# robotics-upo/social_force_window_planner

Measured on AMD Instinct MI355X. Metric: scored trajectories/sec (v x w samples x steps) @ N pedestrians; cmd_vel match, higher is better.
Workload: dtype f64

## Files before the change

include/sfw_hip.h:

```cpp
#ifndef SFW_HIP_H_
#define SFW_HIP_H_

#include <stdint.h>

#ifdef __cplusplus
extern "C" {
#endif

#define SFW_ABI_VERSION 2

typedef enum sfw_status {
  SFW_OK = 0,
  SFW_ERR_INVALID_ARG = -1,
  SFW_ERR_NO_DEVICE = -2,
  SFW_ERR_HIP = -3,
  SFW_ERR_STATE = -4,
  SFW_ERR_UNSUPPORTED = -5
} sfw_status;

#define SFW_COST_INVALID (-1.0)
#define SFW_COST_SKIPPED (-2.0)

#define SFW_ROBOT_ID_NONE INT32_MIN

// ... 128 lines not shown
int sfw_sequences_perturb_stage(sfw_handle h, const sfw_robot_state *rs, const sfw_perturb *p, int32_t n, int32_t K,
                                const int32_t *knot_step, const sfw_goal_args *args, int64_t index_base);
int sfw_score_perturbed(sfw_handle h, const sfw_robot_state *rs, const sfw_perturb *p, int32_t n, int32_t K,
                        const int32_t *knot_step, const sfw_goal_args *args, double *costs_out, sfw_best *best_out);
int sfw_sequences_knots(sfw_handle h, int64_t first, int64_t count, double *vx_out, double *vy_out, double *vtheta_out);
int sfw_sequences_normals(sfw_handle h, int64_t first, int64_t count, double *z_out);

#define SFW_ORG_NONE 0
#define SFW_ORG_REGISTER_1 1
#define SFW_ORG_REGISTER_2 2
#define SFW_ORG_FLAT 3
typedef struct sfw_plan_info {
  int32_t split_step;
  int32_t levels;
  int32_t chunks;
  int32_t organisation;
  int64_t classes;
  int64_t class_steps;
  int64_t samples;
  int64_t flat_samples;
  int64_t one_launch;
  int64_t rest_noise_unreproduced;
} sfw_plan_info;
int sfw_grid_plan_info(sfw_handle h, sfw_plan_info *out);
int sfw_plan_shared_prefix(const double *linvels, int32_t nv,
                           const double *angvels, int32_t nw, double vx0,
                           double vtheta0, double acc_x, double acc_theta,
                           double sim_time, int32_t num_steps,
                           int32_t n_agents, int32_t *level_ends,
                           int64_t *level_classes, int32_t cap,
                           int32_t *n_levels);
int sfw_plan_axis_classes(const double *targets, int32_t n, double v0, double a_max, double dt, int32_t max_p,
                          int32_t form, int32_t *counts, int32_t *classes, int32_t *n_levels, int32_t *closed_form);
int sfw_plan_row_blocks(const double *linvels, int32_t nv, const double *angvels, int32_t nw, double vx0,
                        double vtheta0, double acc_x, double acc_theta, double sim_time, int32_t num_steps,
                        int32_t n_agents, int32_t R, int32_t *row0);
#define SFW_K2_AUTO (-1)
#define SFW_K2_REGISTER 0
#define SFW_K2_FLAT 1
int sfw_set_k2_form(sfw_handle h, int32_t form);
int sfw_set_timing(sfw_handle h, int32_t enabled);
int sfw_last_launch_ms(sfw_handle h, int32_t which, float *ms_out);
int sfw_last_clock_ghz(sfw_handle h, double *ghz_out);
int sfw_grid_points(sfw_handle h, int64_t index, double *points_xyth,
                    int32_t points_cap, int32_t *n_points);
int sfw_grid_points_batch(sfw_handle h, int64_t first, int64_t count, double *points_xyth, int32_t *n_points);
int sfw_set_points_capture(sfw_handle h, int32_t enabled);
void *sfw_stream(sfw_handle h);

#define SFW_TERM_VEL 0
#define SFW_TERM_DISTANCE 1
#define SFW_TERM_ANGLE 2
#define SFW_TERM_COSTMAP 3
#define SFW_TERM_SOCIAL 4
#define SFW_N_TERMS 5
#define SFW_RESCORE_MAX_K 1024
typedef struct sfw_weights {
  double vel, distance, angle, costmap, social;
} sfw_weights;
int sfw_set_terms_capture(sfw_handle h, int32_t enabled);
int sfw_grid_rescore(sfw_handle h, const sfw_weights *w, int32_t K, sfw_best *best_out, double *costs_out);
int sfw_grid_terms(sfw_handle h, int64_t first, int64_t count, double *terms_out);

#define SFW_BLEND_MAX_L 16
typedef struct sfw_blend_stat {
  double lambda;
// ... 120 lines not shown
```

social_force_window_planner_amd/_abi.py:

```python
import ctypes as C

SFW_OK = 0
SFW_ERR_INVALID_ARG = -1
SFW_ERR_NO_DEVICE = -2
SFW_ERR_HIP = -3
SFW_ERR_STATE = -4
SFW_ERR_UNSUPPORTED = -5

SFW_COST_INVALID = -1.0
SFW_COST_SKIPPED = -2.0

SFW_PRECISION_F64 = 0
SFW_PRECISION_F32 = 1
SFW_PRECISION_F64_STRICT = 2

SFW_K2_AUTO, SFW_K2_REGISTER, SFW_K2_FLAT = -1, 0, 1
SFW_ORG_NONE, SFW_ORG_REGISTER_1, SFW_ORG_REGISTER_2, SFW_ORG_FLAT = 0, 1, 2, 3


class SfwParams(C.Structure):
    _fields_ = [
        ("max_vel_x", C.c_double),
        ("sim_time", C.c_double),
        ("sim_granularity", C.c_double),
# ... 104 lines not shown
class SfwPlanInfo(C.Structure):
    _fields_ = [("split_step", C.c_int32), ("levels", C.c_int32), ("chunks", C.c_int32), ("organisation", C.c_int32),
                ("classes", C.c_int64), ("class_steps", C.c_int64), ("samples", C.c_int64), ("flat_samples", C.c_int64),
                ("one_launch", C.c_int64), ("rest_noise_unreproduced", C.c_int64)]

    def as_dict(self):
        return {"split_step": self.split_step, "levels": self.levels, "chunks": self.chunks, "classes": self.classes,
                "class_steps": self.class_steps, "samples": self.samples, "organisation": self.organisation,
                "flat_samples": self.flat_samples, "one_launch": self.one_launch,
                "rest_noise_unreproduced": self.rest_noise_unreproduced}


EXPORTED_SYMBOLS = (
    "sfw_params_default",
    "sfw_abi_version",
    "sfw_create",
    "sfw_destroy",
    "sfw_set_params",
    "sfw_last_error",
    "sfw_set_costmap",
    "sfw_set_footprint",
    "sfw_set_agents",
    "sfw_score_grid",
    "sfw_score_one",
    "sfw_grid_stage",
    "sfw_grid_launch",
    "sfw_grid_sync",
    "sfw_grid_fetch",
    "sfw_grid_costs_view",
    "sfw_grid_plan_info",
    "sfw_plan_shared_prefix",
    "sfw_plan_row_blocks",
    "sfw_plan_axis_classes",
    "sfw_set_k2_form",
    "sfw_set_timing",
    "sfw_last_launch_ms",
    "sfw_last_clock_ghz",
    "sfw_grid_points",
    "sfw_grid_points_batch",
    "sfw_set_points_capture",
    "sfw_stream",
    "sfw_multi_create",
    "sfw_multi_destroy",
    "sfw_multi_last_error",
    "sfw_multi_describe",
    "sfw_multi_ranks",
    "sfw_multi_rank_handle",
    "sfw_multi_set_params",
    "sfw_multi_set_costmap",
    "sfw_multi_set_footprint",
    "sfw_multi_set_agents",
    "sfw_multi_score_grid",
    "sfw_multi_rank_rows",
    "sfw_multi_last_us",
    "sfw_multi_grid_points",
    "sfw_batch_create",
    "sfw_batch_destroy",
    "sfw_batch_last_error",
    "sfw_batch_size",
    "sfw_batch_member",
    "sfw_batch_launch",
    "sfw_batch_fetch",
    "sfw_batch_score_grid",
    "sfw_batch_describe",
    "sfw_batch_last_us",
    "sfw_set_terms_capture",
# ... 121 lines not shown
```

social_force_window_planner_amd/csrc/sfw_capi.hip:

```cpp

#include "sfw_device.h"

#include <dlfcn.h>
#include <link.h>

#include <algorithm>
#include <chrono>
#include <cmath>
#include <condition_variable>
#include <functional>
#include <mutex>
#include <thread>
#include <cstdio>
#include <cstdlib>
#include <cstring>
#include <limits>
#include <new>
#include <string>
#include <vector>

namespace {

template <typename T> struct dev_buf {
  T *p = nullptr;
// ... 32 lines not shown
    return hipEventSynchronize(done);
  }
  hipError_t reserve(size_t bytes) {
    hipError_t e = wait();
    if (e != hipSuccess) return e;
    if (!done && (e = hipEventCreateWithFlags(&done, hipEventDisableTiming)) != hipSuccess) return e;
    if (bytes <= cap) return hipSuccess;
    if (p) (void)hipHostFree(p);
    p = nullptr;
    cap = 0;
    const size_t want = bytes + bytes / 4 + 256;
    e = hipHostMalloc(reinterpret_cast<void **>(&p), want, hipHostMallocDefault);
    if (e == hipSuccess) cap = want;
    return e;
  }
  hipError_t mark(hipStream_t s) {
    pending = true;
    return hipEventRecord(done, s);
  }
  void release() {
    (void)wait();
    if (p) (void)hipHostFree(p);
    if (done) (void)hipEventDestroy(done);
    p = nullptr;
    cap = 0;
    done = nullptr;
  }
};

struct level_tables {
  int32_t n_row = 0, n_col = 0;
  size_t o_row_rep = 0, o_col_rep = 0;
  size_t o_row_src = 0, o_col_src = 0;
};
struct chunk_plan {
  std::vector<level_tables> lv;
  size_t o_row_cls = 0;
};

struct map_geometry {
  uint32_t size_x, size_y;
  double origin_x, origin_y, resolution;
};

struct agent_set {
  std::vector<char> blob;
  size_t ao_vel = 0, ao_cst = 0, ao_obs = 0, ao_grp = 0, ao_off = 0, ao_mem = 0;
  int A = 0, O = 0, NG = 0, n_grp_mem = 0;
  bool person_pinned = false;
  std::vector<std::pair<int32_t, int32_t>> rest_pairs;
};

}

struct sfw_planner_s {
  struct config {
    int n_cu = SFW_DEFAULT_CUS, n_xcd = SFW_DEFAULT_CUS / SFW_CUS_PER_XCD;
    std::vector<int> prefix_env;
    bool pin_rest_on = true;
    long spin_us = 20000;
    bool arena_direct_on = true;
    size_t mirror_max_bytes = size_t(64) << 20;
    int obs_tasks_force = -1;
    size_t table_budget_bytes = size_t(8) << 30;
    bool owns_streams = true;
    bool batch_member = false;
  } cfg;

  struct switches {
    sfw_params params;
// ... 506 lines not shown
  return steps;
}

void plan_row_blocks(const std::vector<double> &lin, const std::vector<double> &ang, double vx0, double vth0, double acc_x,
                     double acc_theta, double dt, int S, int A, int R, int form, int cus, std::vector<int32_t> &row0) {
  const int64_t nv = static_cast<int64_t>(lin.size()), nw = static_cast<int64_t>(ang.size());
  row0.assign(static_cast<size_t>(R) + 1, 0);
  for (int r = 0; r <= R; ++r) row0[static_cast<size_t>(r)] = static_cast<int32_t>((static_cast<int64_t>(r) * nv) / R);
  if (R <= 1 || A < 2 || S < 2 || (nv / R) * nw < 4096) return;
  prefix_classes pc;
  classes_of_grid(pc, lin, ang, vx0, vth0, acc_x, acc_theta, dt, S);
  const std::vector<int> steps = choose_levels(pc, nv * nw, S, static_cast<double>(sfw_samples_per_wave(A, (nv / R) * nw, form, cus)), cus);
  if (steps.empty()) return;
  std::vector<double> w(static_cast<size_t>(nv), static_cast<double>(nw) * (S - steps.back()));
  int prev = 0;
  for (int p : steps) {
    const std::vector<int32_t> &rc = pc.rows.level(p);
    const double per_class = static_cast<double>(pc.n_cols_at(p)) * (p - prev);
    for (int64_t i = 0; i < nv; ++i)
      if (i == 0 || rc[static_cast<size_t>(i)] != rc[static_cast<size_t>(i - 1)]) w[static_cast<size_t>(i)] += per_class;
    prev = p;
  }
  double total = 0.0;
  for (double v : w) total += v;
  double run = 0.0;
  int r = 1;
  for (int64_t i = 0; i < nv && r < R; ++i) {
    run += w[static_cast<size_t>(i)];
    while (r < R && run >= total * r / R) row0[static_cast<size_t>(r++)] = static_cast<int32_t>(i + 1);
  }
  for (; r < R; ++r) row0[static_cast<size_t>(r)] = static_cast<int32_t>(nv);
}

int plan_prefix(sfw_handle h, int64_t chunk, int S) {
  h->st.prefix_steps.clear();
  h->st.prefix_chunks.clear();
  h->st.cls_ints.clear();
  h->st.cls_max = 0;
  h->st.prefix_class_steps = h->st.prefix_last_classes = 0;
  const int64_t T = static_cast<int64_t>(h->st.nv) * h->st.nw;
  const bool forced = !h->cfg.prefix_env.empty();
  if (h->st.list) return SFW_OK;
  if ((forced && h->cfg.prefix_env[0] == 0) || h->st.A < 2 || S < 2 || h->st.vy_samp != 0.0) return SFW_OK;
  if (!forced && T < 4096) return SFW_OK;
  const int64_t rows_per_chunk = chunk / h->st.nw;
  if (rows_per_chunk < 1) return SFW_OK;
  prefix_classes pc;
  classes_of_grid(pc, h->st.lin, h->st.ang, h->st.rs.vx, h->st.rs.vtheta, h->st.ga.acc_x, h->st.ga.acc_theta, h->live.params.sim_time / S, S,
                  static_cast<const axis_classes *>(h->shared_cols));
  const axis_classes &rc = pc.rows, &cc = *pc.cols;
  const std::vector<int32_t> &nr = pc.rows.n, &nc = pc.cols->n;
  auto level = [](const axis_classes &c, int p) -> const std::vector<int32_t> & { return c.level(p); };
  auto count_at = [](const std::vector<int32_t> &n, int p) { return n[std::min<size_t>(static_cast<size_t>(p), n.size()) - 1]; };
  std::vector<int> steps;
  if (forced) {
    for (int p : h->cfg.prefix_env)
      if (p >= 1 && p <= pc.max_p) steps.push_back(p);
  } else {
    steps = choose_levels(pc, T, S, static_cast<double>(sfw_samples_per_wave(h->st.A, std::min<int64_t>(T, rows_per_chunk * h->st.nw), h->live.k2_form, h->cfg.n_cu)), h->cfg.n_cu);
  }
  if (steps.empty()) return SFW_OK;
  const size_t n_lv = steps.size();

  std::vector<int32_t> ints;
  ints.swap(h->st.cls_ints);
  ints.clear();
  ints.reserve(static_cast<size_t>(2 * n_lv + 2) * static_cast<size_t>(h->st.nv + h->st.nw));
  auto append = [&](const std::vector<int32_t> &v) {
    const size_t o = ints.size();
    ints.insert(ints.end(), v.begin(), v.end());
    return o;
  };
  std::vector<int32_t> ids;
  auto relabel = [&ids](const std::vector<int32_t> &cls, int64_t i0, int64_t i1, std::vector<int32_t> &local,
                        std::vector<int32_t> &rep) {
    ids.assign(cls.size(), -1);
    local.clear();
    rep.clear();
    local.reserve(static_cast<size_t>(i1 - i0));
    rep.reserve(static_cast<size_t>(i1 - i0));
    for (int64_t i = i0; i < i1; ++i) {
      int32_t &id = ids[static_cast<size_t>(cls[static_cast<size_t>(i)])];
      if (id < 0) {
        id = static_cast<int32_t>(rep.size());
        rep.push_back(static_cast<int32_t>(i - i0));
      }
      local.push_back(id);
    }
  };
  struct axis_level { std::vector<int32_t> local, rep, src; };
  auto axis_levels = [&](const axis_classes &cls, int64_t i0, int64_t i1) {
    std::vector<axis_level> out(n_lv);
    for (size_t l = 0; l < n_lv; ++l) {
      relabel(level(cls, steps[l]), i0, i1, out[l].local, out[l].rep);
      if (l > 0) {
        out[l].src.reserve(out[l].rep.size());
        for (int32_t r : out[l].rep) out[l].src.push_back(out[l - 1].local[static_cast<size_t>(r)]);
      }
    }
    return out;
  };
  const std::vector<axis_level> cols = axis_levels(cc, 0, h->st.nw);
  std::vector<size_t> o_col_rep(n_lv), o_col_src(n_lv);
  for (size_t l = 0; l < n_lv; ++l) {
    o_col_rep[l] = append(cols[l].rep);
    o_col_src[l] = append(cols[l].src);
  }
  h->st.prefix_o_col_cls = append(cols[n_lv - 1].local);
  int64_t max_cls = 0;
  for (int64_t r0 = 0; r0 < h->st.nv; r0 += rows_per_chunk) {
    const int64_t r1 = std::min<int64_t>(h->st.nv, r0 + rows_per_chunk);
    const std::vector<axis_level> rows = axis_levels(rc, r0, r1);
    chunk_plan cp;
    for (size_t l = 0; l < n_lv; ++l) {
      level_tables t;
      t.n_row = static_cast<int32_t>(rows[l].rep.size());
      t.n_col = static_cast<int32_t>(cols[l].rep.size());
      t.o_row_rep = append(rows[l].rep);
      t.o_row_src = append(rows[l].src);
      t.o_col_rep = o_col_rep[l];
      t.o_col_src = o_col_src[l];
      cp.lv.push_back(t);
      const int64_t n = static_cast<int64_t>(t.n_row) * t.n_col;
      max_cls = std::max(max_cls, n);
      h->st.prefix_class_steps += n * (steps[l] - (l ? steps[l - 1] : 0));
      if (l + 1 == n_lv) h->st.prefix_last_classes += n;
    }
    cp.o_row_cls = append(rows[n_lv - 1].local);
    h->st.prefix_chunks.push_back(cp);
  }
  h->st.cls_ints.swap(ints);
  h->st.cls_max = max_cls;
  h->st.cls_two = n_lv > 1;
  if (std::getenv("SFW_DEBUG_PLAN")) {
    std::fprintf(stderr, "[sfw] shared prefix, %d x %d samples, S=%d, %zu chunk(s):", h->st.nv, h->st.nw, S, h->st.prefix_chunks.size());
    for (size_t l = 0; l < n_lv; ++l)
      std::fprintf(stderr, " [%d,%d) %d x %d;", l ? steps[l - 1] : 0, steps[l], count_at(nr, steps[l]), count_at(nc, steps[l]));
    std::fprintf(stderr, " [%d,%d) samples\n", steps.back(), S);
  }
  h->st.prefix_steps = steps;
  h->st.prefix_S = S;
  h->st.prefix_chunk = rows_per_chunk * h->st.nw;
  return SFW_OK;
}

void rest_forces(const sfw_params &p, const std::vector<std::pair<int32_t, int32_t>> &pairs, const double *pos, const double *vel,
                 int A, double *out) {
  for (int i = 0; i < 2 * A; ++i) out[i] = 0.0;
  for (const auto &pr : pairs) {
    const int i = pr.first, j = pr.second;
    const double dx = pos[2 * j] - pos[2 * i], dy = pos[2 * j + 1] - pos[2 * i + 1];
    const double dn = std::sqrt(dx * dx + dy * dy);
    if (!(dn > 0.0)) continue;
    const double ux = dx / dn, uy = dy / dn;
    const double wx = vel[2 * i] - vel[2 * j], wy = vel[2 * i + 1] - vel[2 * j + 1];
    const double ix = p.sfm_lambda * wx + ux, iy = p.sfm_lambda * wy + uy;
    const double il = std::sqrt(ix * ix + iy * iy);
    if (!(il > 0.0)) continue;
    const double ex = ix / il, ey = iy / il;
    double theta = std::atan2(uy, ux) - std::atan2(ey, ex);
    while (theta <= -M_PI) theta += 2.0 * M_PI;
    while (theta > M_PI) theta -= 2.0 * M_PI;
    const double B = p.sfm_gamma * il;
    if (theta != 0.0) {
      const double sq = p.sfm_n * B * theta;
// ... 604 lines not shown
    L.terms_T = T;
    if (!single && timing) SFW_HIP(h, hipEventRecord(h->chunk_ev[3 * c], h->stream));
    if (prefix) {
      if (!poses_done) SFW_HIP(h, sfw_launch_rollout_poses(L, h->stream));
      SFW_HIP(h, hipEventRecord(h->ev_poses, h->stream));
      if (timing) SFW_HIP(h, hipEventRecord(single ? h->ev[1] : h->chunk_ev[3 * c + 1], h->stream));
      const chunk_plan &cp = h->st.prefix_chunks[static_cast<size_t>(c)];
      const int32_t *tab = h->st.d_cls_tab;
      const size_t n_lv = h->st.prefix_steps.size();
      for (size_t l = 0; l < n_lv; ++l) {
        const level_tables &t = cp.lv[l];
        L.phase = SFW_PHASE_PREFIX;
        L.step_begin = l ? h->st.prefix_steps[l - 1] : 0;
        L.step_end = h->st.prefix_steps[l];
        L.n_cls = t.n_row * t.n_col;
        L.n_col_cls = t.n_col;
        L.row_rep = tab + t.o_row_rep;
        L.col_rep = tab + t.o_col_rep;
        L.resume = l > 0;
        if (l > 0) {
          L.n_col_src = cp.lv[l - 1].n_col;
          L.row_src = tab + t.o_row_src;
          L.col_src = tab + t.o_col_src;
          L.in_state = h->cls_state[(l - 1) & 1].p;
          L.in_dead = h->cls_dead[(l - 1) & 1].p;
        }
        L.out_state = h->cls_state[l & 1].p;
        L.out_dead = h->cls_dead[l & 1].p;
        SFW_HIP(h, launch_social_of(L, h->stream));
      }
      {
        sfw_launch Lc = L;
        Lc.phase = SFW_PHASE_WHOLE;
        SFW_HIP(h, hipStreamWaitEvent(h->side, h->ev_poses, 0));
        SFW_HIP(h, sfw_launch_rollout_costmap(Lc, h->side));
        SFW_HIP(h, hipEventRecord(h->ev_side, h->side));
      }
      SFW_HIP(h, hipStreamWaitEvent(h->stream, h->ev_side, 0));
      L.phase = SFW_PHASE_SUFFIX;
      L.step_begin = h->st.prefix_steps.back();
      L.step_end = S;
      L.resume = 1;
      L.n_col_src = cp.lv[n_lv - 1].n_col;
      L.row_src = tab + cp.o_row_cls;
      L.col_src = tab + h->st.prefix_o_col_cls;
      L.in_state = h->cls_state[(n_lv - 1) & 1].p;
      L.in_dead = h->cls_dead[(n_lv - 1) & 1].p;
      SFW_HIP(h, launch_social_of(L, h->stream, &h->split));
    } else {
      if (!poses_done) SFW_HIP(h, sfw_launch_rollout_poses(L, h->stream));
      SFW_HIP(h, sfw_launch_rollout_costmap(L, h->stream));
      if (timing) SFW_HIP(h, hipEventRecord(single ? h->ev[1] : h->chunk_ev[3 * c + 1], h->stream));
      SFW_HIP(h, launch_social_of(L, h->stream, &h->split));
    }
    if (!single && timing) SFW_HIP(h, hipEventRecord(h->chunk_ev[3 * c + 2], h->stream));
  }
  if (timing) SFW_HIP(h, hipEventRecord(h->ev[2], h->stream));
  SFW_HIP(h, sfw_launch_argmin(h->costs.p, h->st.d_linvels, h->st.d_angvels, h->st.nw, T, h->st.index_base,
                               h->partials.p, h->st.d_sel, h->stream, costs_host, sel_host, h->st.list));
  if (timing) SFW_HIP(h, hipEventRecord(h->ev[3], h->stream));
  h->last.timed = timing;
  ++h->launch_seq;
  h->last.launched = true;
  return SFW_OK;
}

hipError_t launch_cycle_of(const sfw_launch &L, hipStream_t stream) {
  return L.p.precision == SFW_PRECISION_F64_STRICT ? sfw_launch_cycle_strict(L, stream) : sfw_launch_cycle(L, stream);
// ... 811 lines not shown
      (cap > 0 && (!level_ends || !level_classes)))
    return SFW_ERR_INVALID_ARG;
  *n_levels = 0;
  const int64_t T = static_cast<int64_t>(nv) * nw;
  if (n_agents < 2 || num_steps < 2 || T < 4096) return SFW_OK;
  const std::vector<double> lin(linvels, linvels + nv), ang(angvels, angvels + nw);
  prefix_classes pc;
  classes_of_grid(pc, lin, ang, vx0, vtheta0, acc_x, acc_theta, sim_time / num_steps, num_steps);
  const int cus = env_device_cus(SFW_DEFAULT_CUS);
  const std::vector<int> steps = choose_levels(pc, T, num_steps, static_cast<double>(sfw_samples_per_wave(n_agents, T, SFW_K2_AUTO, cus)), cus);
  *n_levels = static_cast<int32_t>(steps.size());
  for (size_t l = 0; l < steps.size() && l < static_cast<size_t>(cap); ++l) {
    level_ends[l] = steps[l];
    level_classes[l] = static_cast<int64_t>(pc.n_rows_at(steps[l])) * pc.n_cols_at(steps[l]);
  }
  return SFW_OK;
}

int sfw_plan_axis_classes(const double *targets, int32_t n, double v0, double a_max, double dt, int32_t max_p, int32_t form,
                          int32_t *counts, int32_t *classes, int32_t *n_levels, int32_t *closed_form) {
  if (!targets || n <= 0 || max_p < 1 || !counts || !n_levels || (form != 0 && form != 1)) return SFW_ERR_INVALID_ARG;
  if (!all_finite(targets, static_cast<size_t>(n)) || !std::isfinite(v0) || !std::isfinite(a_max) || !std::isfinite(dt))
    return SFW_ERR_INVALID_ARG;
  const axis_classes a = classes_of_axis(std::vector<double>(targets, targets + n), v0, a_max, dt, max_p, form == 0);
  *n_levels = static_cast<int32_t>(a.n.size());
  if (closed_form) *closed_form = a.fast ? 1 : 0;
  for (size_t l = 0; l < a.n.size(); ++l) {
    counts[l] = a.n[l];
    if (classes) std::memcpy(classes + l * static_cast<size_t>(n), a.level(static_cast<int>(l) + 1).data(), sizeof(int32_t) * static_cast<size_t>(n));
  }
  return SFW_OK;
}

int sfw_plan_row_blocks(const double *linvels, int32_t nv, const double *angvels, int32_t nw, double vx0, double vtheta0,
                        double acc_x, double acc_theta, double sim_time, int32_t num_steps, int32_t n_agents, int32_t R,
                        int32_t *row0) {
  if (!linvels || !angvels || nv <= 0 || nw <= 0 || num_steps < 1 || R < 1 || !row0) return SFW_ERR_INVALID_ARG;
  if (!all_finite(linvels, static_cast<size_t>(nv)) || !all_finite(angvels, static_cast<size_t>(nw))) return SFW_ERR_INVALID_ARG;
  const std::vector<double> lin(linvels, linvels + nv), ang(angvels, angvels + nw);
  std::vector<int32_t> cuts;
  plan_row_blocks(lin, ang, vx0, vtheta0, acc_x, acc_theta, sim_time / num_steps, num_steps, n_agents, R, SFW_K2_AUTO,
                  env_device_cus(SFW_DEFAULT_CUS), cuts);
  std::memcpy(row0, cuts.data(), sizeof(int32_t) * (static_cast<size_t>(R) + 1));
  return SFW_OK;
}

int sfw_grid_plan_info(sfw_handle h, sfw_plan_info *out) {
  if (!h || !out) return SFW_ERR_INVALID_ARG;
  if (!h->st.valid) return fail(h, SFW_ERR_STATE, "grid_plan_info before grid_stage");
  const int64_t T = static_cast<int64_t>(h->st.nv) * h->st.nw;
  out->split_step = h->st.prefix_steps.empty() ? 0 : h->st.prefix_steps.back();
  out->levels = static_cast<int32_t>(h->st.prefix_steps.size());
  out->samples = T;
  out->classes = h->st.prefix_last_classes;
  out->class_steps = h->st.prefix_class_steps;
  if (!h->st.prefix_steps.empty()) {
    out->chunks = static_cast<int32_t>(h->st.prefix_chunks.size());
  } else {
    int64_t chunk = h->st.table_chunk;
    if (chunk > T) chunk = T;
    out->chunks = chunk > 0 ? static_cast<int32_t>((T + chunk - 1) / chunk) : 0;
  }
  out->organisation = sfw_social_organisation(h->st.A, out->chunks > 0 ? (T + out->chunks - 1) / out->chunks : T, h->st.O, h->live.k2_form, h->cfg.n_cu);
  out->flat_samples = sfw_social_flat_items(h->st.A, h->st.O, h->st.NG, out->chunks > 0 ? (T + out->chunks - 1) / out->chunks : T, h->live.k2_form, h->cfg.n_cu);
  out->rest_noise_unreproduced = rest_noise_unreproduced(h) ? 1 : 0;
  out->one_launch = 0;
// ... 1646 lines not shown
```

social_force_window_planner_amd/csrc/sfw_device.h:

```cpp
#ifndef SFW_DEVICE_H_
#define SFW_DEVICE_H_

#include <hip/hip_runtime.h>
#include <stdint.h>

#include "../../include/sfw_hip.h"


#define SFW_DEFAULT_CUS 256
#define SFW_CUS_PER_XCD 32

enum : int32_t { SFW_ST_VALID = 0, SFW_ST_INVALID = 1, SFW_ST_SKIPPED = 2 };

struct __attribute__((aligned(32))) sfw_robot_step {
  double x, y, vx, vy;
};

struct __attribute__((aligned(32))) sfw_pose_frame {
  double x, y, c, s;
};

struct __attribute__((aligned(16))) sfw_unit {
  double a, b;
};
// ... 113 lines not shown
  const char *arena_host;
  char *arena_dev;
  uint32_t arena_bytes;
  double *terms;
  int64_t terms_T;
  const double *vy_samps;
  int32_t list;
  int32_t n_knots;
  const int32_t *knot_step;
  int64_t knot_stride;
};

__device__ __forceinline__ void sfw_put_term(double *terms, int64_t T, int64_t t, int k, double v) {
  if (terms) terms[k * T + t] = v;
}
__device__ __forceinline__ void sfw_put_terms3(double *terms, int64_t T, int64_t t, double vel, double d, double ang) {
  if (!terms) return;
  terms[SFW_TERM_VEL * T + t] = vel;
  terms[SFW_TERM_DISTANCE * T + t] = d;
  terms[SFW_TERM_ANGLE * T + t] = ang;
}
__device__ __forceinline__ void sfw_put_terms_sentinel(double *terms, int64_t T, int64_t t, double sentinel) {
  if (!terms) return;
  for (int k = 0; k < SFW_N_TERMS; ++k) terms[k * T + t] = sentinel;
}


struct sfw_crowd_out {
  double *state;
  double *work;
  int32_t *has_goal;
};

void sfw_derive(sfw_launch &L);

hipError_t sfw_launch_rollout(const sfw_launch &L, hipStream_t stream);
hipError_t sfw_launch_rollout_poses(const sfw_launch &L, hipStream_t stream);
hipError_t sfw_launch_rollout_costmap(const sfw_launch &L, hipStream_t stream);
struct sfw_split_streams {
  hipStream_t side;
  hipEvent_t fork, join;
};
hipError_t sfw_launch_social(const sfw_launch &L, hipStream_t stream, const sfw_split_streams *sp = nullptr);
bool sfw_cycle_applies(const sfw_launch &L);
hipError_t sfw_launch_cycle(const sfw_launch &L, hipStream_t stream);
struct sfw_batch_rec {
  sfw_launch L;
  int32_t k2_bytes;
  int32_t lds_bytes;
};
inline size_t sfw_batch_recs_offset(int B) { return (sizeof(uint32_t) * (static_cast<size_t>(B) + 1) + 15) & ~size_t(15); }
int sfw_cycle_batch_variant(const sfw_launch &L);
void sfw_cycle_batch_record(const sfw_launch &L, sfw_batch_rec *rec);
hipError_t sfw_launch_cycle_batch(int variant, const uint32_t *d_first, const sfw_batch_rec *d_recs, int B, unsigned blocks,
                                  size_t lds, hipStream_t stream);
#ifndef SFW_STRICT_BUILD
hipError_t sfw_launch_cycle_batch_strict(int variant, const uint32_t *d_first, const sfw_batch_rec *d_recs, int B,
                                         unsigned blocks, size_t lds, hipStream_t stream);
int64_t sfw_social_flat_items(int A, int O, int NG, int64_t T, int form, int cus);
hipError_t sfw_launch_social_strict(const sfw_launch &L, hipStream_t stream, const sfw_split_streams *sp = nullptr);
hipError_t sfw_launch_cycle_strict(const sfw_launch &L, hipStream_t stream);
hipError_t sfw_launch_crowd_strict(const sfw_launch &L, const sfw_crowd_out &cw, hipStream_t stream);
#endif
hipError_t sfw_launch_crowd(const sfw_launch &L, const sfw_crowd_out &cw, hipStream_t stream);
bool sfw_rollout_is_fused(const sfw_launch &L);
int64_t sfw_argmin_partials(int64_t T);
hipError_t sfw_launch_argmin(const double *costs, const double *linvels, const double *angvels,
                             int32_t nw, int64_t T, int64_t index_base, sfw_sel *partials,
                             sfw_sel *out, hipStream_t stream, double *costs_host = nullptr,
                             sfw_sel *sel_host = nullptr, bool list = false);
int64_t sfw_rescore_blocks(int64_t T, int K);
// ... 58 lines not shown
```

social_force_window_planner_amd/csrc/sfw_kernels.hip:

```cpp

#include "sfw_device.h"
#include "sfw_math.h"

#include <type_traits>

#include <limits.h>
#include <math.h>
#include <stdlib.h>
#include <cmath>

namespace {

constexpr int WAVE = 64;

#pragma clang fp contract(off)

__device__ __forceinline__ unsigned cell_index(double a, double res, double inv_res) {
  const double q = a * inv_res;
  const double m = __builtin_trunc(q);
  const double d = q - m;
  if (d < 1e-9 || d > 1.0 - 1e-9) return static_cast<unsigned>(a / res);
  return static_cast<unsigned>(m);
}

// ... 341 lines not shown
  const int64_t n = L.chunk_count;
  if (idx >= n * L.S) return;
  const int64_t step = idx / n, local = idx - step * n;
  if (L.status[L.chunk_begin + local] == SFW_ST_SKIPPED) return;
  const sfw_unit pos = step == 0 ? sfw_unit{L.rs.x, L.rs.y} : L.ptab[(step - 1) * L.row_units + local];
  const sfw_unit cs = LIST ? L.cs_tab[step * L.rstep_stride + local] : L.cs_tab[step * L.nw + (L.chunk_begin + local) % L.nw];
  const double fc = footprint_cost(L, pos.a, pos.b, cs.a, cs.b);
  L.fcode[step * L.rstep_stride + local] = static_cast<int16_t>(fc);
}

__global__ void __launch_bounds__(256) sfw_costmap_scan_kernel(const sfw_launch L) {
  const int64_t local = static_cast<int64_t>(blockIdx.x) * blockDim.x + threadIdx.x;
  if (local >= L.chunk_count) return;
  const int64_t t = L.chunk_begin + local;
  if (L.status[t] == SFW_ST_SKIPPED) {
    if (L.n_points) L.n_points[local] = 0;
    return;
  }
  const int S = L.S;
  double cm = 0.0;
  int n_ok = 0;
  bool stopped = false;
  for (int base = 0; base < S && !stopped; base += 8) {
    int16_t v[8];
#pragma unroll
    for (int j = 0; j < 8; ++j)
      v[j] = (base + j < S) ? L.fcode[static_cast<int64_t>(base + j) * L.rstep_stride + local] : int16_t(-1);
#pragma unroll
    for (int j = 0; j < 8; ++j)
      if (!stopped && base + j < S) stopped = !scan_code(static_cast<double>(v[j]), cm, n_ok);
  }
  scan_finish(L, t, local, cm, n_ok);
}

constexpr int FOOT_OFFMAP = 300;
__device__ __forceinline__ int footprint_edge(const sfw_launch &L, double x, double y, double c, double s, int e) {
  const double inv_res = 1.0 / L.resolution;
  const int e1 = (e + 1 < L.K) ? e + 1 : 0;
  const double ax = L.footprint[2 * e], ay = L.footprint[2 * e + 1], bx = L.footprint[2 * e1], by = L.footprint[2 * e1 + 1];
  unsigned x0, y0, x1, y1;
  if (!world_to_map(L, inv_res, x + (ax * c - ay * s), y + (ax * s + ay * c), x0, y0)) return FOOT_OFFMAP;
  if (!world_to_map(L, inv_res, x + (bx * c - by * s), y + (bx * s + by * c), x1, y1)) return FOOT_OFFMAP;
  return line_max(L, (int)x0, (int)y0, (int)x1, (int)y1);
}

constexpr int K1_SMALL_MAX_STEPS = 512;
constexpr int K1_SMALL_BLOCK = 256;
struct k1s_lds {
  double *th, *vxs, *vys;
  double2 *cs, *dxy;
  double *xs, *ys;
  int *code;
  double *quot;
  double *th_end;
  __host__ __device__ k1s_lds(char *base, int S, size_t *bytes = nullptr) {
    char *const base0 = base;
    auto take = [&](size_t n) {
      char *p = base;
      base += (n + 15) & ~size_t(15);
      return p;
    };
    const size_t n = static_cast<size_t>(S);
    th = reinterpret_cast<double *>(take(8 * n));
    vxs = reinterpret_cast<double *>(take(8 * n));
    vys = reinterpret_cast<double *>(take(8 * n));
    cs = reinterpret_cast<double2 *>(take(16 * n));
// ... 2414 lines not shown
                       dim3(static_cast<unsigned>(L.chunk_count)), dim3(K1_SMALL_BLOCK), 0, stream, L);
    return hipGetLastError();
  }
  const int block = 64;
  if (sfw_k1a_threads()) {
    const unsigned grid = static_cast<unsigned>((L.chunk_count + block - 1) / block);
    hipLaunchKernelGGL((L.n_knots > 1 ? sfw_rollout_kernel<true, true> : L.list ? sfw_rollout_kernel<true> : sfw_rollout_kernel<false>),
                       dim3(grid), dim3(block), 0, stream, L);
    return hipGetLastError();
  }
  constexpr int per_wave = WAVE / K1A_TEAM;
  const unsigned grid = static_cast<unsigned>((L.chunk_count + per_wave - 1) / per_wave);
  hipLaunchKernelGGL((L.n_knots > 1 ? sfw_rollout_team_kernel<true, true> : L.list ? sfw_rollout_team_kernel<true> : sfw_rollout_team_kernel<false>),
                     dim3(grid), dim3(block), 0, stream, L);
  return hipGetLastError();
}

hipError_t sfw_launch_rollout_costmap(const sfw_launch &L, hipStream_t stream) {
  if (L.chunk_count <= 0 || sfw_rollout_is_fused(L)) return hipSuccess;
  {
    const int block = 256;
    const int64_t n = L.chunk_count * L.S;
    const unsigned grid = static_cast<unsigned>((n + block - 1) / block);
    hipLaunchKernelGGL((L.list ? sfw_footprint_kernel<true> : sfw_footprint_kernel<false>), dim3(grid), dim3(block), 0, stream, L);
  }
  {
    const int block = 256;
    const unsigned grid = static_cast<unsigned>((L.chunk_count + block - 1) / block);
    hipLaunchKernelGGL(sfw_costmap_scan_kernel, dim3(grid), dim3(block), 0, stream, L);
  }
  return hipGetLastError();
}

hipError_t sfw_launch_rollout(const sfw_launch &L, hipStream_t stream) {
  hipError_t e = sfw_launch_rollout_poses(L, stream);
  return e != hipSuccess ? e : sfw_launch_rollout_costmap(L, stream);
}

template <typename K> static hipError_t launch_social_as(K kernel, const sfw_launch &L, int G, unsigned grid,
                                                          size_t lds, hipStream_t stream) {
  if (lds > 64 * 1024) {
    hipError_t e = hipFuncSetAttribute(reinterpret_cast<const void *>(kernel),
                                       hipFuncAttributeMaxDynamicSharedMemorySize, static_cast<int>(lds));
    if (e != hipSuccess) return e;
  }
  hipLaunchKernelGGL(kernel, dim3(grid), dim3(WAVE), lds, stream, L, G);
  return hipGetLastError();
}

template <int CAP> static bool reg_layout_matches() {
  const lds_layout s(nullptr, 5, CAP, 10, 2, 3, 0, 0, true, false);
  auto at = [&](const void *p) { return static_cast<int>(reinterpret_cast<const char *>(p) - reinterpret_cast<const char *>(s.px)); };
  using off = reg_off<CAP>;
  return at(s.py) == off::PY && at(s.vx) == off::VX && at(s.vy) == off::VY && at(s.fjx) == off::FJX && at(s.fjy) == off::FJY &&
         at(s.hasgoal) == off::HG && at(s.swp) == off::SW && at(s.dead) == off::DEAD && at(s.rsb) == off::RSB && s.hg_stride == 2;
}

static int64_t split_point(const wave_plan &pl, int A, int O, int NG, int form, int64_t items, int cus) {
  if (form != SFW_K2_AUTO || pl.flat || pl.ns != 1 || A < 2 || A > WAVE || NG > 0) return items;
  const int64_t S = 4LL * cus, W = (items + pl.G - 1) / pl.G, q = W / S;
  if (q < 1 || q > 5 || W % S == 0) return items;
  const int64_t reg_items = q * S * pl.G, rest = items - reg_items;
  const int P = A * (A - 1) / 2, Lseg = (O + OBS_SEG - 1) / OBS_SEG;
  const double c_reg_wave = 90.0 * (A / 2) + 225.0 + 24.0 * O;
  const double c_flat_wave = 1.03 * (85.0 * ((P + WAVE - 1) / WAVE) + 215.0) + 24.7 * ((A + OBS_AGENT_LANES - 1) / OBS_AGENT_LANES) * Lseg;
  const double t_now = static_cast<double>(q + 1), t_split = q + static_cast<double>((rest + S - 1) / S) * c_flat_wave / c_reg_wave;
// ... 398 lines not shown
```

Baseline: 7.591 million.

## Compute footprint costs once per shared-prefix class instead of per trajectory

During the shared-prefix phase, trajectories within a class share identical poses, so the footprint kernel now evaluates the footprint cost only for class representatives and stores codes in a compact per-level table. The scan kernel maps each trajectory to its class code for prefix steps and reads per-trajectory codes afterward. This is meant to cut redundant footprint/line-raster work for early steps, at the cost of indirection lookups in the scan and extra host-side tables. A host planning API exposes the tables for testing.

```diff
diff --git a/include/sfw_hip.h b/include/sfw_hip.h
--- a/include/sfw_hip.h
+++ b/include/sfw_hip.h
@@ -184,6 +184,11 @@
                            int32_t *n_levels);
 int sfw_plan_axis_classes(const double *targets, int32_t n, double v0, double a_max, double dt, int32_t max_p,
                           int32_t form, int32_t *counts, int32_t *classes, int32_t *n_levels, int32_t *closed_form);
+int sfw_plan_footprint_tables(const double *linvels, int32_t nv, const double *angvels, int32_t nw, double vx0,
+                              double vtheta0, double acc_x, double acc_theta, double sim_time, int32_t num_steps,
+                              const int32_t *level_ends, int32_t n_levels, int32_t rows_per_chunk, int32_t *tab,
+                              int64_t tab_cap, int64_t *tab_len, int64_t *chunk_records, int32_t chunk_cap,
+                              int32_t *n_chunks);
 int sfw_plan_row_blocks(const double *linvels, int32_t nv, const double *angvels, int32_t nw, double vx0,
                         double vtheta0, double acc_x, double acc_theta, double sim_time, int32_t num_steps,
                         int32_t n_agents, int32_t R, int32_t *row0);
diff --git a/social_force_window_planner_amd/_abi.py b/social_force_window_planner_amd/_abi.py
--- a/social_force_window_planner_amd/_abi.py
+++ b/social_force_window_planner_amd/_abi.py
@@ -160,6 +160,7 @@
     "sfw_plan_shared_prefix",
     "sfw_plan_row_blocks",
     "sfw_plan_axis_classes",
+    "sfw_plan_footprint_tables",
     "sfw_set_k2_form",
     "sfw_set_timing",
     "sfw_last_launch_ms",
diff --git a/social_force_window_planner_amd/csrc/sfw_capi.hip b/social_force_window_planner_amd/csrc/sfw_capi.hip
--- a/social_force_window_planner_amd/csrc/sfw_capi.hip
+++ b/social_force_window_planner_amd/csrc/sfw_capi.hip
@@ -88,10 +88,13 @@
   int32_t n_row = 0, n_col = 0;
   size_t o_row_rep = 0, o_col_rep = 0;
   size_t o_row_src = 0, o_col_src = 0;
+  size_t o_row_map = 0, o_col_map = 0;
 };
 struct chunk_plan {
   std::vector<level_tables> lv;
   size_t o_row_cls = 0;
+  size_t o_fp_lv = 0;
+  int32_t fp_blocks = 0;
 };
 
 struct map_geometry {
@@ -664,40 +667,23 @@
   for (; r < R; ++r) row0[static_cast<size_t>(r)] = static_cast<int32_t>(nv);
 }
 
-int plan_prefix(sfw_handle h, int64_t chunk, int S) {
-  h->st.prefix_steps.clear();
-  h->st.prefix_chunks.clear();
-  h->st.cls_ints.clear();
-  h->st.cls_max = 0;
-  h->st.prefix_class_steps = h->st.prefix_last_classes = 0;
-  const int64_t T = static_cast<int64_t>(h->st.nv) * h->st.nw;
-  const bool forced = !h->cfg.prefix_env.empty();
-  if (h->st.list) return SFW_OK;
-  if ((forced && h->cfg.prefix_env[0] == 0) || h->st.A < 2 || S < 2 || h->st.vy_samp != 0.0) return SFW_OK;
-  if (!forced && T < 4096) return SFW_OK;
-  const int64_t rows_per_chunk = chunk / h->st.nw;
-  if (rows_per_chunk < 1) return SFW_OK;
-  prefix_classes pc;
-  classes_of_grid(pc, h->st.lin, h->st.ang, h->st.rs.vx, h->st.rs.vtheta, h->st.ga.acc_x, h->st.ga.acc_theta, h->live.params.sim_time / S, S,
-                  static_cast<const axis_classes *>(h->shared_cols));
+struct prefix_tables {
+  std::vector<int32_t> ints;
+  std::vector<chunk_plan> chunks;
+  size_t o_col_cls = 0;
+  int64_t max_cls = 0, class_steps = 0, last_classes = 0;
+};
+void build_prefix_tables(const prefix_classes &pc, const std::vector<int> &steps, int64_t nv, int64_t nw, int64_t rows_per_chunk,
+                         prefix_tables &pt) {
+  const size_t n_lv = steps.size();
+
+  std::vector<int32_t> &ints = pt.ints;
+  ints.clear();
+  pt.chunks.clear();
+  pt.max_cls = pt.class_steps = pt.last_classes = 0;
   const axis_classes &rc = pc.rows, &cc = *pc.cols;
-  const std::vector<int32_t> &nr = pc.rows.n, &nc = pc.cols->n;
   auto level = [](const axis_classes &c, int p) -> const std::vector<int32_t> & { return c.level(p); };
-  auto count_at = [](const std::vector<int32_t> &n, int p) { return n[std::min<size_t>(static_cast<size_t>(p), n.size()) - 1]; };
-  std::vector<int> steps;
-  if (forced) {
-    for (int p : h->cfg.prefix_env)
-      if (p >= 1 && p <= pc.max_p) steps.push_back(p);
-  } else {
-    steps = choose_levels(pc, T, S, static_cast<double>(sfw_samples_per_wave(h->st.A, std::min<int64_t>(T, rows_per_chunk * h->st.nw), h->live.k2_form, h->cfg.n_cu)), h->cfg.n_cu);
-  }
-  if (steps.empty()) return SFW_OK;
-  const size_t n_lv = steps.size();
-
-  std::vector<int32_t> ints;
-  ints.swap(h->st.cls_ints);
-  ints.clear();
-  ints.reserve(static_cast<size_t>(2 * n_lv + 2) * static_cast<size_t>(h->st.nv + h->st.nw));
+  ints.reserve(static_cast<size_t>(3 * n_lv + 2) * static_cast<size_t>(nv + nw) + n_lv * SFW_FP_LV_INTS * static_cast<size_t>((nv + rows_per_chunk - 1) / rows_per_chunk));
   auto append = [&](const std::vector<int32_t> &v) {
     const size_t o = ints.size();
     ints.insert(ints.end(), v.begin(), v.end());
@@ -732,16 +718,17 @@
     }
     return out;
   };
-  const std::vector<axis_level> cols = axis_levels(cc, 0, h->st.nw);
+  const std::vector<axis_level> cols = axis_levels(cc, 0, nw);
   std::vector<size_t> o_col_rep(n_lv), o_col_src(n_lv);
   for (size_t l = 0; l < n_lv; ++l) {
     o_col_rep[l] = append(cols[l].rep);
     o_col_src[l] = append(cols[l].src);
   }
-  h->st.prefix_o_col_cls = append(cols[n_lv - 1].local);
-  int64_t max_cls = 0;
-  for (int64_t r0 = 0; r0 < h->st.nv; r0 += rows_per_chunk) {
-    const int64_t r1 = std::min<int64_t>(h->st.nv, r0 + rows_per_chunk);
+  pt.o_col_cls = append(cols[n_lv - 1].local);
+  std::vector<size_t> o_col_map(n_lv);
+  for (size_t l = 0; l < n_lv; ++l) o_col_map[l] = l + 1 < n_lv ? append(cols[l].local) : pt.o_col_cls;
+  for (int64_t r0 = 0; r0 < nv; r0 += rows_per_chunk) {
+    const int64_t r1 = std::min<int64_t>(nv, r0 + rows_per_chunk);
     const std::vector<axis_level> rows = axis_levels(rc, r0, r1);
     chunk_plan cp;
     for (size_t l = 0; l < n_lv; ++l) {
@@ -754,15 +741,76 @@
       t.o_col_src = o_col_src[l];
       cp.lv.push_back(t);
       const int64_t n = static_cast<int64_t>(t.n_row) * t.n_col;
-      max_cls = std::max(max_cls, n);
-      h->st.prefix_class_steps += n * (steps[l] - (l ? steps[l - 1] : 0));
-      if (l + 1 == n_lv) h->st.prefix_last_classes += n;
+      pt.max_cls = std::max(pt.max_cls, n);
+      pt.class_steps += n * (steps[l] - (l ? steps[l - 1] : 0));
+      if (l + 1 == n_lv) pt.last_classes += n;
     }
     cp.o_row_cls = append(rows[n_lv - 1].local);
-    h->st.prefix_chunks.push_back(cp);
-  }
-  h->st.cls_ints.swap(ints);
-  h->st.cls_max = max_cls;
+    int64_t code_off = 0, blk = 0;
+    std::vector<int32_t> rec(n_lv * SFW_FP_LV_INTS, 0);
+    for (size_t l = 0; l < n_lv; ++l) {
+      level_tables &t = cp.lv[l];
+      t.o_row_map = l + 1 < n_lv ? append(rows[l].local) : cp.o_row_cls;
+      t.o_col_map = o_col_map[l];
+      const int s0 = l ? steps[l - 1] : 0, s1 = l + 1 < n_lv ? steps[l] : steps[l] + 1;
+      int32_t *const r = rec.data() + l * SFW_FP_LV_INTS;
+      r[SFW_FP_S0] = s0;
+      r[SFW_FP_S1] = s1;
+      r[SFW_FP_N_ROW] = t.n_row;
+      r[SFW_FP_N_COL] = t.n_col;
+      r[SFW_FP_ROW_REP] = static_cast<int32_t>(t.o_row_rep);
+      r[SFW_FP_COL_REP] = static_cast<int32_t>(t.o_col_rep);
+      r[SFW_FP_ROW_MAP] = static_cast<int32_t>(t.o_row_map);
+      r[SFW_FP_COL_MAP] = static_cast<int32_t>(t.o_col_map);
+      r[SFW_FP_CODE_LO] = static_cast<int32_t>(static_cast<uint32_t>(code_off & 0xffffffff));
+      r[SFW_FP_CODE_HI] = static_cast<int32_t>(code_off >> 32);
+      r[SFW_FP_BLK0] = static_cast<int32_t>(blk);
+      const int64_t poses = static_cast<int64_t>(t.n_row) * t.n_col * (s1 - s0);
+      code_off += poses;
+      blk += (poses + SFW_FP_BLOCK - 1) / SFW_FP_BLOCK;
+    }
+    cp.o_fp_lv = append(rec);
+    cp.fp_blocks = static_cast<int32_t>(blk);
+    pt.chunks.push_back(cp);
+  }
+}
+
+int plan_prefix(sfw_handle h, int64_t chunk, int S) {
+  h->st.prefix_steps.clear();
+  h->st.prefix_chunks.clear();
+  h->st.cls_ints.clear();
+  h->st.cls_max = 0;
+  h->st.prefix_class_steps = h->st.prefix_last_classes = 0;
+  const int64_t T = static_cast<int64_t>(h->st.nv) * h->st.nw;
+  const bool forced = !h->cfg.prefix_env.empty();
+  if (h->st.list) return SFW_OK;
+  if ((forced && h->cfg.prefix_env[0] == 0) || h->st.A < 2 || S < 2 || h->st.vy_samp != 0.0) return SFW_OK;
+  if (!forced && T < 4096) return SFW_OK;
+  const int64_t rows_per_chunk = chunk / h->st.nw;
+  if (rows_per_chunk < 1) return SFW_OK;
+  prefix_classes pc;
+  classes_of_grid(pc, h->st.lin, h->st.ang, h->st.rs.vx, h->st.rs.vtheta, h->st.ga.acc_x, h->st.ga.acc_theta, h->live.params.sim_time / S, S,
+                  static_cast<const axis_classes *>(h->shared_cols));
+  const std::vector<int32_t> &nr = pc.rows.n, &nc = pc.cols->n;
+  auto count_at = [](const std::vector<int32_t> &n, int p) { return n[std::min<size_t>(static_cast<size_t>(p), n.size()) - 1]; };
+  std::vector<int> steps;
+  if (forced) {
+    for (int p : h->cfg.prefix_env)
+      if (p >= 1 && p <= pc.max_p) steps.push_back(p);
+  } else {
+    steps = choose_levels(pc, T, S, static_cast<double>(sfw_samples_per_wave(h->st.A, std::min<int64_t>(T, rows_per_chunk * h->st.nw), h->live.k2_form, h->cfg.n_cu)), h->cfg.n_cu);
+  }
+  if (steps.empty()) return SFW_OK;
+  const size_t n_lv = steps.size();
+  prefix_tables pt;
+  pt.ints.swap(h->st.cls_ints);
+  build_prefix_tables(pc, steps, h->st.nv, h->st.nw, rows_per_chunk, pt);
+  h->st.prefix_chunks.swap(pt.chunks);
+  h->st.prefix_o_col_cls = pt.o_col_cls;
+  h->st.prefix_class_steps = pt.class_steps;
+  h->st.prefix_last_classes = pt.last_classes;
+  h->st.cls_ints.swap(pt.ints);
+  h->st.cls_max = pt.max_cls;
   h->st.cls_two = n_lv > 1;
   if (std::getenv("SFW_DEBUG_PLAN")) {
     std::fprintf(stderr, "[sfw] shared prefix, %d x %d samples, S=%d, %zu chunk(s):", h->st.nv, h->st.nw, S, h->st.prefix_chunks.size());
@@ -1433,8 +1481,14 @@
       {
         sfw_launch Lc = L;
         Lc.phase = SFW_PHASE_WHOLE;
+        sfw_fp_plan fp;
+        fp.lv = tab + cp.o_fp_lv;
+        fp.tab = tab;
+        fp.n_lv = static_cast<int32_t>(n_lv);
+        fp.shared_end = h->st.prefix_steps.back() + 1;
+        fp.shared_blocks = cp.fp_blocks;
         SFW_HIP(h, hipStreamWaitEvent(h->side, h->ev_poses, 0));
-        SFW_HIP(h, sfw_launch_rollout_costmap(Lc, h->side));
+        SFW_HIP(h, sfw_launch_rollout_costmap_shared(Lc, fp, h->side));
         SFW_HIP(h, hipEventRecord(h->ev_side, h->side));
       }
       SFW_HIP(h, hipStreamWaitEvent(h->stream, h->ev_side, 0));
@@ -2312,6 +2366,31 @@
   return SFW_OK;
 }
 
+int sfw_plan_footprint_tables(const double *linvels, int32_t nv, const double *angvels, int32_t nw, double vx0, double vtheta0,
+                              double acc_x, double acc_theta, double sim_time, int32_t num_steps, const int32_t *level_ends,
+                              int32_t n_levels, int32_t rows_per_chunk, int32_t *tab, int64_t tab_cap, int64_t *tab_len,
+                              int64_t *chunk_records, int32_t chunk_cap, int32_t *n_chunks) {
+  if (!linvels || !angvels || nv <= 0 || nw <= 0 || num_steps < 2 || !level_ends || n_levels < 1 || rows_per_chunk < 1 || !tab_len ||
+      !n_chunks || tab_cap < 0 || chunk_cap < 0 || (tab_cap > 0 && !tab) || (chunk_cap > 0 && !chunk_records))
+    return SFW_ERR_INVALID_ARG;
+  if (!all_finite(linvels, static_cast<size_t>(nv)) || !all_finite(angvels, static_cast<size_t>(nw))) return SFW_ERR_INVALID_ARG;
+  std::vector<int> steps(level_ends, level_ends + n_levels);
+  for (int32_t l = 0; l < n_levels; ++l)
+    if (steps[static_cast<size_t>(l)] < 1 || steps[static_cast<size_t>(l)] > prefix_max_p(num_steps) ||
+        (l && steps[static_cast<size_t>(l)] <= steps[static_cast<size_t>(l - 1)]))
+      return SFW_ERR_INVALID_ARG;
+  const std::vector<double> lin(linvels, linvels + nv), ang(angvels, angvels + nw);
+  prefix_classes pc;
+  classes_of_grid(pc, lin, ang, vx0, vtheta0, acc_x, acc_theta, sim_time / num_steps, num_steps);
+  prefix_tables pt;
+  build_prefix_tables(pc, steps, nv, nw, rows_per_chunk, pt);
+  *tab_len = static_cast<int64_t>(pt.ints.size());
+  *n_chunks = static_cast<int32_t>(pt.chunks.size());
+  if (tab_cap >= *tab_len) std::memcpy(tab, pt.ints.data(), sizeof(int32_t) * pt.ints.size());
+  for (size_t c = 0; c < pt.chunks.size() && c < static_cast<size_t>(chunk_cap); ++c) chunk_records[c] = static_cast<int64_t>(pt.chunks[c].o_fp_lv);
+  return SFW_OK;
+}
+
 int sfw_plan_row_blocks(const double *linvels, int32_t nv, const double *angvels, int32_t nw, double vx0, double vtheta0,
                         double acc_x, double acc_theta, double sim_time, int32_t num_steps, int32_t n_agents, int32_t R,
                         int32_t *row0) {
diff --git a/social_force_window_planner_amd/csrc/sfw_device.h b/social_force_window_planner_amd/csrc/sfw_device.h
--- a/social_force_window_planner_amd/csrc/sfw_device.h
+++ b/social_force_window_planner_amd/csrc/sfw_device.h
@@ -169,11 +169,35 @@
   int32_t *has_goal;
 };
 
+enum {
+  SFW_FP_S0 = 0,
+  SFW_FP_S1,
+  SFW_FP_N_ROW,
+  SFW_FP_N_COL,
+  SFW_FP_ROW_REP,
+  SFW_FP_COL_REP,
+  SFW_FP_ROW_MAP,
+  SFW_FP_COL_MAP,
+  SFW_FP_CODE_LO,
+  SFW_FP_CODE_HI,
+  SFW_FP_BLK0,
+  SFW_FP_LV_INTS = 12
+};
+constexpr int SFW_FP_BLOCK = 256;
+struct sfw_fp_plan {
+  const int32_t *lv;
+  const int32_t *tab;
+  int32_t n_lv;
+  int32_t shared_end;
+  int32_t shared_blocks;
+};
+
 void sfw_derive(sfw_launch &L);
 
 hipError_t sfw_launch_rollout(const sfw_launch &L, hipStream_t stream);
 hipError_t sfw_launch_rollout_poses(const sfw_launch &L, hipStream_t stream);
 hipError_t sfw_launch_rollout_costmap(const sfw_launch &L, hipStream_t stream);
+hipError_t sfw_launch_rollout_costmap_shared(const sfw_launch &L, const sfw_fp_plan &fp, hipStream_t stream);
 struct sfw_split_streams {
   hipStream_t side;
   hipEvent_t fork, join;
diff --git a/social_force_window_planner_amd/csrc/sfw_kernels.hip b/social_force_window_planner_amd/csrc/sfw_kernels.hip
--- a/social_force_window_planner_amd/csrc/sfw_kernels.hip
+++ b/social_force_window_planner_amd/csrc/sfw_kernels.hip
@@ -397,6 +397,84 @@
   }
   scan_finish(L, t, local, cm, n_ok);
 }
+
+#ifndef SFW_STRICT_BUILD
+__global__ void __launch_bounds__(SFW_FP_BLOCK) sfw_footprint_shared_kernel(const sfw_launch L, const sfw_fp_plan fp) {
+  const int64_t n = L.chunk_count;
+  const int blk = static_cast<int>(blockIdx.x);
+  if (blk >= fp.shared_blocks) {
+    const int64_t idx = static_cast<int64_t>(blk - fp.shared_blocks) * SFW_FP_BLOCK + threadIdx.x;
+    if (idx >= n * (L.S - fp.shared_end)) return;
+    const int64_t q = idx / n, local = idx - q * n, step = fp.shared_end + q;
+    if (L.status[L.chunk_begin + local] == SFW_ST_SKIPPED) return;
+    const sfw_unit pos = L.ptab[(step - 1) * L.row_units + local];
+    const sfw_unit cs = L.cs_tab[step * L.nw + (L.chunk_begin + local) % L.nw];
+    const double fc = footprint_cost(L, pos.a, pos.b, cs.a, cs.b);
+    L.fcode[step * L.rstep_stride + local] = static_cast<int16_t>(fc);
+    return;
+  }
+  int l = 0;
+  while (l + 1 < fp.n_lv && blk >= fp.lv[(l + 1) * SFW_FP_LV_INTS + SFW_FP_BLK0]) ++l;
+  const int32_t *const lv = fp.lv + l * SFW_FP_LV_INTS;
+  const int s0 = lv[SFW_FP_S0], n_col = lv[SFW_FP_N_COL];
+  const int64_t n_cls = static_cast<int64_t>(lv[SFW_FP_N_ROW]) * n_col;
+  const int64_t j = static_cast<int64_t>(blk - lv[SFW_FP_BLK0]) * SFW_FP_BLOCK + threadIdx.x;
+  if (j >= n_cls * (lv[SFW_FP_S1] - s0)) return;
+  const int64_t q = j / n_cls, cls = j - q * n_cls, step = s0 + q;
+  const int r = static_cast<int>(cls / n_col), c = static_cast<int>(cls - static_cast<int64_t>(r) * n_col);
+  const int col = fp.tab[lv[SFW_FP_COL_REP] + c];
+  const int64_t local = static_cast<int64_t>(fp.tab[lv[SFW_FP_ROW_REP] + r]) * L.nw + col;
+  const sfw_unit pos = step == 0 ? sfw_unit{L.rs.x, L.rs.y} : L.ptab[(step - 1) * L.row_units + local];
+  const sfw_unit cs = L.cs_tab[step * L.nw + col];
+  const double fc = footprint_cost(L, pos.a, pos.b, cs.a, cs.b);
+  const int64_t code_off = static_cast<int64_t>(static_cast<uint32_t>(lv[SFW_FP_CODE_LO])) | (static_cast<int64_t>(lv[SFW_FP_CODE_HI]) << 32);
+  L.fcode[code_off + j] = static_cast<int16_t>(fc);
+}
+
+__global__ void __launch_bounds__(256) sfw_costmap_scan_shared_kernel(const sfw_launch L, const sfw_fp_plan fp) {
+  const int64_t local = static_cast<int64_t>(blockIdx.x) * blockDim.x + threadIdx.x;
+  if (local >= L.chunk_count) return;
+  const int64_t t = L.chunk_begin + local;
+  if (L.status[t] == SFW_ST_SKIPPED) {
+    if (L.n_points) L.n_points[local] = 0;
+    return;
+  }
+  const int S = L.S;
+  const int row = static_cast<int>(local / L.nw), col = static_cast<int>(local - static_cast<int64_t>(row) * L.nw);
+  double cm = 0.0;
+  int n_ok = 0;
+  bool stopped = false;
+  int l = -1, lv_s0 = 0, lv_s1 = 0;
+  int64_t lv_cls = 0, lv_code = 0;
+  for (int base = 0; base < S && !stopped; base += 8) {
+    int16_t v[8];
+#pragma unroll
+    for (int j = 0; j < 8; ++j) {
+      const int step = base + j;
+      if (step >= S) {
+        v[j] = int16_t(-1);
+      } else if (step < fp.shared_end) {
+        while (step >= lv_s1 && l + 1 < fp.n_lv) {
+          const int32_t *const lv = fp.lv + ++l * SFW_FP_LV_INTS;
+          lv_s0 = lv[SFW_FP_S0];
+          lv_s1 = lv[SFW_FP_S1];
+          const int n_col = lv[SFW_FP_N_COL];
+          lv_cls = static_cast<int64_t>(lv[SFW_FP_N_ROW]) * n_col;
+          const int64_t code_off = static_cast<int64_t>(static_cast<uint32_t>(lv[SFW_FP_CODE_LO])) | (static_cast<int64_t>(lv[SFW_FP_CODE_HI]) << 32);
+          lv_code = code_off + static_cast<int64_t>(fp.tab[lv[SFW_FP_ROW_MAP] + row]) * n_col + fp.tab[lv[SFW_FP_COL_MAP] + col];
+        }
+        v[j] = L.fcode[lv_code + (step - lv_s0) * lv_cls];
+      } else {
+        v[j] = L.fcode[static_cast<int64_t>(step) * L.rstep_stride + local];
+      }
+    }
+#pragma unroll
+    for (int j = 0; j < 8; ++j)
+      if (!stopped && base + j < S) stopped = !scan_code(static_cast<double>(v[j]), cm, n_ok);
+  }
+  scan_finish(L, t, local, cm, n_ok);
+}
+#endif
 
 constexpr int FOOT_OFFMAP = 300;
 __device__ __forceinline__ int footprint_edge(const sfw_launch &L, double x, double y, double c, double s, int e) {
@@ -2877,6 +2955,24 @@
   return hipGetLastError();
 }
 
+#ifndef SFW_STRICT_BUILD
+hipError_t sfw_launch_rollout_costmap_shared(const sfw_launch &L, const sfw_fp_plan &fp, hipStream_t stream) {
+  if (L.chunk_count <= 0 || sfw_rollout_is_fused(L)) return hipSuccess;
+  if (L.list || fp.n_lv < 1 || fp.shared_end < 1 || fp.shared_end > L.S) return hipErrorInvalidValue;
+  {
+    const int64_t own = L.chunk_count * (L.S - fp.shared_end);
+    const unsigned grid = static_cast<unsigned>(fp.shared_blocks + (own + SFW_FP_BLOCK - 1) / SFW_FP_BLOCK);
+    hipLaunchKernelGGL(sfw_footprint_shared_kernel, dim3(grid), dim3(SFW_FP_BLOCK), 0, stream, L, fp);
+  }
+  {
+    const int block = 256;
+    const unsigned grid = static_cast<unsigned>((L.chunk_count + block - 1) / block);
+    hipLaunchKernelGGL(sfw_costmap_scan_shared_kernel, dim3(grid), dim3(block), 0, stream, L, fp);
+  }
+  return hipGetLastError();
+}
+#endif
+
 hipError_t sfw_launch_rollout(const sfw_launch &L, hipStream_t stream) {
   hipError_t e = sfw_launch_rollout_poses(L, stream);
   return e != hipSuccess ? e : sfw_launch_rollout_costmap(L, stream);
```

Result: no change. 7.599 million (median of 2 runs) (+0.1%).
